# eddyxzc/lpopc

Measured on AMD Instinct MI355X. Metric: eval_g+eval_jac_g calls/sec, 4-phase 4096-LGR-pt problem, higher is better.
Workload: dtype f64

## Files before the change

lpopc_amd/csrc/rpm_ipm_device.hpp:

```cpp
#pragma once
#include <hip/hip_runtime.h>

#include "rpm_ipm.hpp"

namespace rpm {

constexpr int IPM_FMAX = 1024;
constexpr int IPM_TRACE = 8;
constexpr double IPM_INF = 1e19;
constexpr int IPM_LB_H = 6;
constexpr int IPM_LB_PART = 80 * 16;
constexpr int IPM_LB_SMALL = 8 + 2 * (2 * IPM_LB_H) * (2 * IPM_LB_H) + 2 * (2 * IPM_LB_H);

struct IpmOpts {
  double tol = 1e-8, mu_init = 0.1, kappa_eps = 10.0, kappa_mu = 0.2, theta_mu = 1.5, tau_min = 0.99;
  double bound_push = 1e-2, bound_frac = 1e-2, kappa_sigma = 1e10, s_max = 100.0;
  double ws_bound_push = 1e-3, ws_bound_frac = 1e-3, ws_slack_bound_push = 1e-3, ws_slack_bound_frac = 1e-3;
  double ws_mult_bound_push = 1e-3, ws_mult_init_max = 1e6;
  double gamma_theta = 1e-5, gamma_phi = 1e-8, eta_phi = 1e-8, delta = 1.0, s_theta = 1.1, s_phi = 2.3, gamma_alpha = 0.05;
  double delta_c = 1e-9, delta_w_first = 1e-4, delta_w_min = 1e-20, delta_w_max = 1e40, kw_inc_first = 100.0, kw_inc = 8.0,
         kw_dec = 1.0 / 3.0;
  int max_iter = 3000, max_ls = 40;
  double acceptable_tol = 1e-6;
  int acceptable_iter = 15;
// ... 35 lines not shown
struct IpmDev {
  int B, n, m, ns, nv, Nt, Nb, nb, b, CS, nnz_jac, nnz_h;
  long long sg, sv, kstride;
  const int *pos, *row_slack, *slack_row, *jac_dst, *hes_dst, *diag_dst, *slk_dst, *jt_ptr, *jt_ent, *jt_row;
  const int *hg_ptr, *hg_src, *hg_dst;
  int n_hg;
  const int *as_dst, *as_ki, *as_hg, *as_ptr;
  int as_nchunk;
  const int* long_cols;
  int n_long;
  const double *gl, *gu;
  double *v, *vl, *vu, *zL, *zU, *lam, *dv, *dlam, *dzL, *dzU, *glag, *c, *rhs, *K, *filt;
  double *xe, *xt, *grad, *g, *jac, *hess, *obj, *gt, *objt;
  double *vR, *dr2;
  double *vl0, *vu0;
  double *pp, *nn, *zp, *zn, *dpp, *dnn, *dzp, *dzn;
  double* rfilt;
  double* part;
  int* tick;
  double *dv2, *dlam2, *dzL2, *dzU2, *csoc, *ct;
  double* trace;
  int trace_cap;
  IpmInst* inst;
  int* cnt;
  IpmOpts o;
  const KktSub* subs;
  int n_sub, n_l1, n_l2;
  int* piv;
  const int *cg_ptr, *cg_src, *cg_dst;
  const int *rg_ptr, *rg_src, *rg_dst;
  const int *rs_dst, *rs_src;
  const int* gap_pos;
  int n_cg, n_rg, n_rs, n_gap;
  const int *cg2_ptr, *cg2_src, *cg2_dst, *rg2_ptr, *rg2_src, *rg2_dst, *rs2_dst, *rs2_src;
  int n_cg2, n_rg2, n_rs2;
  int n_cg_long, n_cg2_long;
  int max_sub_nt;
  int df_tiles;
  size_t l1_dense_lds;
  int last_dense_corner;
  size_t l2_dense_lds, last_dense_lds;
  int df_on;
  const int *df_ptr, *df_ki, *df_hg, *as_live;
  int as_nlive;
  const unsigned long long* df_map;
  int rhs_mult;
  int lb_on;
  double *lb_S, *lb_Y;
  double *lb_xprev;
  double *lb_gold;
  int scal_on;
  double *sc, *sf, *lam_h;
  const int* jac_row;
  int nnz_var;
  double *lb_small;
  double *lb_part;
  double *lb_Z;
};

constexpr int IPM_VEC_BLOCKS = 64;
constexpr int IPM_VEC_PART = 24;
constexpr int IPM_MT = 8;

void ipm_launch_set_state0(const IpmDev& D, int x_state0, int M, int nx, const double* d_state0, hipStream_t st);
void ipm_launch_init(const IpmDev& D, const double* d_x0, hipStream_t st, int warm = 0);
void ipm_launch_init_slack(const IpmDev& D, hipStream_t st, int warm = 0);
void ipm_launch_warm_duals(const IpmDev& D, const double* d_x0, const double* d_lambda, const double* d_zL, const double* d_zU, hipStream_t st);
void ipm_launch_bound_multipliers(const IpmDev& D, double* d_zL, double* d_zU, hipStream_t st);
void ipm_launch_pack_x(const IpmDev& D, hipStream_t st);
void ipm_launch_residual(const IpmDev& D, hipStream_t st);
void ipm_launch_assemble(const IpmDev& D, int nnz_max, hipStream_t st);
void ipm_launch_inertia(const IpmDev& D, hipStream_t st);
void ipm_launch_direction(const IpmDev& D, hipStream_t st);
void ipm_launch_trial(const IpmDev& D, hipStream_t st);
void ipm_launch_accept(const IpmDev& D, hipStream_t st);
void ipm_launch_update(const IpmDev& D, hipStream_t st);
void ipm_launch_soc_rhs(const IpmDev& D, hipStream_t st);
void ipm_launch_soc_direction(const IpmDev& D, hipStream_t st);
void ipm_launch_scaling_factors(const IpmDev& D, hipStream_t st);
void ipm_launch_scale(const IpmDev& D, double* g, double* jac, int jac0, int jac1, double* obj, double* grad, hipStream_t st);
void ipm_launch_scale_lambda(const IpmDev& D, hipStream_t st);
void ipm_launch_scale_hessian(const IpmDev& D, hipStream_t st);
void ipm_launch_unscale_lambda(const IpmDev& D, double* out, hipStream_t st);
void lb_launch_reset(const IpmDev& D, hipStream_t st);
void lb_launch_update(const IpmDev& D, hipStream_t st);
void lb_launch_columns_and_solve(const IpmDev& D, hipStream_t st);
// ... 15 lines not shown
```

lpopc_amd/csrc/rpm_ipm_solver.hip:

```cpp
#include <algorithm>
#include <cstdlib>
#include <cstring>
#include <memory>
#include <new>

#include "rpm_ipm_solver.hpp"

using namespace rpm;

namespace {
struct IpmAllocs {
  rpm_ipm* h;
  int rc = RPM_OK;
  template <class T>
  void room(T** dst, size_t count) { if (!rc) rc = ipm_alloc(h, dst, count); }
  template <class T>
  void table(const T** dst, const std::vector<T>& src) {
    T* p = nullptr;
    if (!rc) rc = ipm_alloc(h, &p, src.size(), src.data());
    *dst = p;
  }
};

bool env_is_zero(const char* name) {
// ... 45 lines not shown
  D.n_cg = int(p.cg_dst.size()); D.n_rg = int(p.rg_dst.size()); D.n_rs = int(p.rs_dst.size()); D.n_gap = int(p.gap_pos.size());
  a.table(&D.cg2_ptr, p.cg2_ptr); a.table(&D.cg2_src, p.cg2_src); a.table(&D.cg2_dst, p.cg2_dst);
  a.table(&D.rg2_ptr, p.rg2_ptr); a.table(&D.rg2_src, p.rg2_src); a.table(&D.rg2_dst, p.rg2_dst);
  a.table(&D.rs2_dst, p.rs2_dst); a.table(&D.rs2_src, p.rs2_src);
  D.n_cg2 = int(p.cg2_dst.size()); D.n_rg2 = int(p.rg2_dst.size()); D.n_rs2 = int(p.rs2_dst.size());
  D.n_cg_long = p.n_cg_long; D.n_cg2_long = p.n_cg2_long;
  return a.rc;
}

int alloc_state(rpm_ipm* h) {
  Engine& e = h->eng->e;
  const IpmPlan& p = h->plan;
  IpmDev& D = h->D;
  const size_t B = size_t(D.B), Bm = B * size_t(std::max(p.m, 1));
  IpmAllocs a{h};
  a.room(&D.v, B * p.nv); a.room(&D.vl, B * p.nv); a.room(&D.vu, B * p.nv);
  a.room(&D.zL, B * p.nv); a.room(&D.zU, B * p.nv); a.room(&D.lam, B * p.m);
  a.room(&D.dv, B * p.nv); a.room(&D.dlam, B * p.m); a.room(&D.dzL, B * p.nv);
  a.room(&D.dzU, B * p.nv); a.room(&D.glag, B * p.nv); a.room(&D.c, B * p.m);
  a.room(&D.rhs, B * size_t(p.Nt_alloc)); a.room(&D.K, B * size_t(p.storage())); a.room(&D.filt, B * 2 * IPM_FMAX);
  a.room(&D.xe, B * p.n); a.room(&D.xt, B * p.n); a.room(&D.grad, B * p.n);
  a.room(&D.g, B * size_t(D.sg)); a.room(&D.jac, B * size_t(D.sv)); a.room(&D.hess, B * size_t(e.nnz_h));
  a.room(&D.obj, B); a.room(&D.gt, B * size_t(D.sg)); a.room(&D.objt, B);
  a.room(&D.inst, B); a.room(&D.cnt, size_t(4));
  a.room(&D.vR, B * p.nv); a.room(&D.dr2, B * p.nv);
  a.room(&D.vl0, B * p.nv); a.room(&D.vu0, B * p.nv);
  if (h->lbfgs) {
    a.room(&D.lb_S, B * IPM_LB_H * p.n); a.room(&D.lb_Y, B * IPM_LB_H * p.n);
    a.room(&D.lb_xprev, B * p.n); a.room(&D.lb_gold, B * p.nv);
    a.room(&D.lb_small, B * IPM_LB_SMALL); a.room(&D.lb_part, B * IPM_LB_PART);
    a.room(&D.lb_Z, size_t(2 * IPM_LB_H) * B * size_t(p.Nt_alloc));
  }
  a.room(&D.sc, Bm); a.room(&D.sf, B); a.room(&D.lam_h, Bm);
  a.table(&D.jac_row, e.jac_i);
  D.nnz_var = e.nnz_nl + e.nnz_lin;
  a.room(&D.pp, Bm); a.room(&D.nn, Bm); a.room(&D.zp, Bm); a.room(&D.zn, Bm);
  a.room(&D.dpp, Bm); a.room(&D.dnn, Bm); a.room(&D.dzp, Bm); a.room(&D.dzn, Bm);
  a.room(&D.dlam2, Bm); a.room(&D.csoc, Bm); a.room(&D.ct, Bm);
  a.room(&D.dv2, B * p.nv); a.room(&D.dzL2, B * p.nv); a.room(&D.dzU2, B * p.nv);
  a.room(&D.rfilt, B * 2 * IPM_FMAX);
  a.room(&D.part, B * IPM_VEC_BLOCKS * IPM_VEC_PART); a.room(&D.tick, B);
  if (a.rc) return a.rc;
  if (hipMemsetAsync(D.tick, 0, B * sizeof(int), static_cast<hipStream_t>(dev_stream(e))) != hipSuccess) return device_failed(h, "hipMemset");
  if (hipHostMalloc(reinterpret_cast<void**>(&h->h_cnt), 4 * sizeof(int)) != hipSuccess) return device_failed(h, "hipHostMalloc");
  std::vector<double> l(B * p.nv, 0.0), u(B * p.nv, 0.0);
  for (size_t bi = 0; bi < B; ++bi)
    for (int i = 0; i < p.n; ++i) { l[bi * p.nv + i] = e.xl[i]; u[bi * p.nv + i] = e.xu[i]; }
  if (hipMemcpy(D.vl0, l.data(), l.size() * sizeof(double), hipMemcpyHostToDevice) != hipSuccess ||
      hipMemcpy(D.vu0, u.data(), u.size() * sizeof(double), hipMemcpyHostToDevice) != hipSuccess) return device_failed(h, "hipMemcpy");
  h->h_inst.resize(B);
  return RPM_OK;
}

int choose_kernels(rpm_ipm* h, const IpmSubList& s) {
  const IpmPlan& p = h->plan;
  IpmDev& D = h->D;
  const size_t B = size_t(D.B);
  D.last_dense_corner = 1;
  if (s.n_l1 > 0) {
    auto dense_lds_of = [&](int first, int count) -> size_t {
      int rows = 0;
      for (int i = first; i < first + count; ++i) rows = std::max(rows, s.subs[size_t(i)].g.block_rows());
      return count > 0 && rows <= kkt_factor_dense_max_block_rows() ? kkt_factor_dense_lds_bytes(rows) : 0;
    };
    h->l1_dense_lds = dense_lds_of(0, s.n_l1);
    h->l2_dense_lds = dense_lds_of(s.n_l1, s.n_l2);
    for (int i = s.n_l1; i < s.n_l1 + s.n_l2; ++i)
// ... 14 lines not shown
  if (p.max_rows > 4 * IPM_MT * 16) {
    h->err = "band + border of " + std::to_string(p.max_rows - IPM_W) + " rows exceeds the factorisation's 512 rows per block column";
    return RPM_E_UNSUPPORTED;
  }
  h->factor_lds = kkt_factor_lds_bytes(p);
  if (h->factor_lds > 150 * 1024) {
    h->err = "band of " + std::to_string(p.b) + " and border of " + std::to_string(p.nb) + " rows do not fit the factorisation's LDS";
    return RPM_E_UNSUPPORTED;
  }
  if (kkt_factor_prepare(h->factor_mt, h->factor_lds) != hipSuccess) return device_failed(h, "hipFuncSetAttribute");
  return RPM_OK;
}
}

extern "C" {

int rpm_ipm_create(rpm_engine* eng, rpm_ipm** out) {
  if (!eng || !out) return RPM_E_INVALID;
  *out = nullptr;
  Engine& e = eng->e;
  const bool lbfgs = e.hessian_mode != RPM_HESSIAN_EXACT;
  if (e.shard_world > 1) {
    e.err = "rpm_ipm_create: interval-sharded engines are not supported (shard instances across ranks instead)";
    return RPM_E_UNSUPPORTED;
  }
  if (!e.dev) {
    int rc = device_init(e, 0);
    if (rc) return rc;
  }
  int rc = lbfgs ? RPM_OK : ensure_hessian(e);
  if (rc) return rc;
  std::unique_ptr<rpm_ipm> h(new (std::nothrow) rpm_ipm);
  if (!h) return RPM_E_INVALID;
  h->eng = eng;
  h->lbfgs = lbfgs;
  e.ipm_attached += 1;
  h->attached = true;
  auto fail = [&e](int code, const std::string& why) { e.err = "rpm_ipm_create: " + why; return code; };

  std::string why;
  rc = build_ipm_plan(e, h->plan, &why, e.opt_ipm_nested != 0);
  if (e.opt_ipm_nested == -1 && (rc || h->plan.max_rows > 4 * IPM_MT * 16 || kkt_factor_lds_bytes(h->plan) > 150 * 1024))
    rc = build_ipm_plan(e, h->plan, &why, 0);
  if (rc) return fail(rc, why);
  const IpmPlan& p = h->plan;

// ... 411 lines not shown
```

lpopc_amd/csrc/rpm_ipm_solver.hpp:

```cpp
#pragma once
#include <algorithm>
#include <cstdio>
#include <string>
#include <vector>

#include "rpm_device_internal.hpp"
#include "rpm_ipm_device.hpp"

struct rpm_ipm {
  rpm_engine* eng = nullptr;
  rpm::IpmPlan plan;
  rpm::IpmDev D{};
  std::vector<void*> allocs;
  int* h_cnt = nullptr;
  size_t factor_lds = 0;
  size_t l1_dense_lds = 0;
  size_t l2_dense_lds = 0, last_dense_lds = 0;
  int factor_mt = rpm::IPM_MT;
  std::string err;
  std::vector<rpm::IpmInst> h_inst;
  int total_factorizations = 0, total_iterations = 0, total_trials = 0, total_soc = 0;
  hipEvent_t ev[4] = {nullptr, nullptr, nullptr, nullptr};
  double factor_ms = 0.0, solve_ms = 0.0;
  bool solve_pending = false;
// ... 46 lines not shown
  if (factor) kkt_launch_factor(h->D, h->factor_mt, h->factor_lds, st);
  if (solve) kkt_launch_solve(h->D, check_status, st, forward_done);
  return launch_check(h, "kkt kernels");
}

int ipm_check_start_args(rpm_ipm* h, const char* who, const char* need, bool warm, const void* x, const void* lambda, const void* z_L,
                         const void* z_U);
int ipm_start(rpm_ipm* h, bool warm, const double* d_x, const double* d_lambda, const double* d_zL, const double* d_zU, hipStream_t st);
int host_form(rpm_ipm* h, double** d_x, double** d_l, double** d_zL, double** d_zU);

inline int ipm_abi_status(int device_status) {
  return device_status == 1 ? 0 : (device_status == 6 ? 1 : device_status);
}

struct IpmLoop {
  rpm_ipm* h;
  Engine& e;
  IpmDev& D;
  hipStream_t st;
  bool scal;
  int eng_fail(int rc) const { h->err = e.err; return rc; }

  int fetch_counts() const {
    IPM_TRY(h, hipMemcpyAsync(h->h_cnt, D.cnt, 4 * sizeof(int), hipMemcpyDeviceToHost, st));
    IPM_TRY(h, hipStreamSynchronize(st));
    return RPM_OK;
  }
  int evaluate_and_residual() const {
    int rc;
    ipm_launch_pack_x(D, st);
    if ((rc = dev_eval_obj(e, D.xe, D.obj, D.grad, st))) return eng_fail(rc);
    if ((rc = dev_eval_cons(e, D.xe, D.g, D.jac, 3 | 4 | 16, st))) return eng_fail(rc);
    if (scal) ipm_launch_scale(D, D.g, D.jac, 0, D.nnz_var, D.obj, D.grad, st);
    IPM_TRY(h, hipMemsetAsync(D.cnt, 0, 4 * sizeof(int), st));
    ipm_launch_residual(D, st);
    if (h->lbfgs) lb_launch_update(D, st);
    return fetch_counts();
  }
  int exact_hessian() const {
    if (scal) ipm_launch_scale_lambda(D, st);
    if (int rc = dev_eval_h(e, D.xe, 1.0, scal ? D.lam_h : D.lam, D.hess, st)) return eng_fail(rc);
    if (scal) ipm_launch_scale_hessian(D, st);
    return RPM_OK;
  }
  int factor_with_inertia_correction() const {
    int rc;
    for (int tries = 0; tries < 80; ++tries) {
      IPM_TRY(h, hipMemsetAsync(D.cnt + 1, 0, sizeof(int), st));
      ipm_launch_assemble(D, std::max(e.nnz_jac, e.nnz_h), st);
      IPM_TRY(h, hipEventRecord(h->ev[0], st));
      if ((rc = factor_and_solve_launch(h, st, true, false, 1))) return rc;
      IPM_TRY(h, hipEventRecord(h->ev[1], st));
      ipm_launch_inertia(D, st);
      h->total_factorizations += 1;
      if ((rc = fetch_counts())) return rc;
      float ms = 0.f;
      if (hipEventElapsedTime(&ms, h->ev[0], h->ev[1]) == hipSuccess) h->factor_ms += ms;
      if (h->h_cnt[1] == 0) break;
    }
    return RPM_OK;
  }
  int substitute() const {
    IPM_TRY(h, hipEventRecord(h->ev[2], st));
    if (h->lbfgs && h->lb_iterations > 0) {
      lb_launch_columns_and_solve(D, st);
      lb_launch_small(D, st);
    }
    if (int rc = factor_and_solve_launch(h, st, false, true, 1, 1)) return rc;
    if (h->lbfgs) lb_launch_correct(D, 1, st);
    IPM_TRY(h, hipEventRecord(h->ev[3], st));
    h->solve_pending = true;
    return RPM_OK;
  }
  int direction() const {
    IPM_TRY(h, hipMemsetAsync(D.cnt + 2, 0, 2 * sizeof(int), st));
    ipm_launch_direction(D, st);
    h->h_cnt[3] = 0;
    return RPM_OK;
  }
  int line_search_round(double* soc_rhs_copy = nullptr) const {
    int rc;
    if (h->h_cnt[3] > 0) {
      ipm_launch_soc_rhs(D, st);
      if (soc_rhs_copy)
        IPM_TRY(h, hipMemcpyAsync(soc_rhs_copy, D.rhs, size_t(D.B) * size_t(h->plan.Nt_alloc) * sizeof(double), hipMemcpyDeviceToHost, st));
      if ((rc = factor_and_solve_launch(h, st, false, true, 2))) return rc;
      if (h->lbfgs) lb_launch_correct(D, 2, st);
      ipm_launch_soc_direction(D, st);
      h->total_soc += 1;
    }
    ipm_launch_trial(D, st);
    if ((rc = dev_eval_obj(e, D.xt, D.objt, nullptr, st))) return eng_fail(rc);
    if ((rc = dev_eval_cons(e, D.xt, D.gt, nullptr, 1 | 4, st))) return eng_fail(rc);
    if (scal) ipm_launch_scale(D, D.gt, nullptr, 0, 0, D.objt, nullptr, st);
    IPM_TRY(h, hipMemsetAsync(D.cnt + 2, 0, 2 * sizeof(int), st));
    ipm_launch_accept(D, st);
    h->total_trials += 1;
    if ((rc = fetch_counts())) return rc;
    if (h->solve_pending) {
      float ms = 0.f;
      if (hipEventElapsedTime(&ms, h->ev[2], h->ev[3]) == hipSuccess) h->solve_ms += ms;
      h->solve_pending = false;
    }
    return RPM_OK;
  }
  bool line_search_over() const { return h->h_cnt[2] == 0 && h->h_cnt[3] == 0; }
  int line_search() const {
    int rc;
    if ((rc = direction())) return rc;
    for (int ls = 0; ls <= D.o.max_ls + D.o.max_soc + 2; ++ls) {
      if ((rc = line_search_round())) return rc;
      if (line_search_over()) break;
    }
    return RPM_OK;
  }
  int update() const {
    ipm_launch_update(D, st);
    if (h->lbfgs) {
// ... 39 lines not shown
```

lpopc_amd/csrc/rpm_ipm_step_kernels.hip:

```cpp
#include <algorithm>
#include <cmath>
#include <cstring>
#include <new>

#include "rpm_device_internal.hpp"
#include "rpm_ipm_device.hpp"

namespace rpm {

__device__ inline double block_red(double v, int kind, double* sh) {
  for (int o = 32; o; o >>= 1) {
    const double w = __shfl_down(v, o);
    v = kind == 0 ? v + w : (kind == 1 ? fmax(v, w) : fmin(v, w));
  }
  __syncthreads();
  if ((threadIdx.x & 63) == 0) sh[threadIdx.x >> 6] = v;
  __syncthreads();
  double r = sh[0];
  for (int i = 1; i < int(blockDim.x >> 6); ++i) r = kind == 0 ? r + sh[i] : (kind == 1 ? fmax(r, sh[i]) : fmin(r, sh[i]));
  return r;
}
__device__ inline bool has_lo(double l, double u) { return l > -IPM_INF && l != u; }
__device__ inline bool has_up(double l, double u) { return u < IPM_INF && l != u; }

// ... 214 lines not shown
  if (S.status != 0) return;
  const double *lam = D.lam + size_t(bi) * D.m, *jac = D.jac + size_t(bi) * D.sv;
  const bool resto = S.mode == 2;
  if (int(blockIdx.x) >= n_thread_blocks) {
    const int i = D.long_cols[blockIdx.x - n_thread_blocks];
    double acc = 0.0;
    for (int q = D.jt_ptr[i] + threadIdx.x; q < D.jt_ptr[i + 1]; q += blockDim.x) acc += jac[D.jt_ent[q]] * lam[D.jt_row[q]];
    acc = block_red(acc, 0, sh);
    if (threadIdx.x == 0) D.glag[size_t(bi) * D.nv + i] = (resto ? 0.0 : D.grad[size_t(bi) * D.n + i]) + acc;
    return;
  }
  const int i = blockIdx.x * blockDim.x + threadIdx.x;
  if (i >= D.nv) return;
  double acc;
  if (i < D.n) {
    if (D.jt_ptr[i + 1] - D.jt_ptr[i] > IPM_LONG_COLUMN) return;
    acc = resto ? 0.0 : D.grad[size_t(bi) * D.n + i];
    for (int q = D.jt_ptr[i]; q < D.jt_ptr[i + 1]; ++q) acc += jac[D.jt_ent[q]] * lam[D.jt_row[q]];
  } else {
    acc = -lam[D.slack_row[i - D.n]];
  }
  D.glag[size_t(bi) * D.nv + i] = acc;
}
__global__ __launch_bounds__(1024) void ipm_residual_kernel(IpmDev D) {
  __shared__ double sh[16];
  __shared__ int verdict;
  const int bi = blockIdx.y, t = threadIdx.x, i0 = blockIdx.x * blockDim.x + threadIdx.x, stride = gridDim.x * blockDim.x;
  IpmInst& S = D.inst[bi];
  if (S.status != 0) return;
  const int mode_in = S.mode;
  if (mode_in == 3) {
    if (t == 0 && blockIdx.x == 0) { S.refactor = 1; S.delta_w = 0.0; atomicAdd(&D.cnt[0], 1); }
    return;
  }
  const double *v = D.v + size_t(bi) * D.nv, *vl = D.vl + size_t(bi) * D.nv, *vu = D.vu + size_t(bi) * D.nv;
  const double *zL = D.zL + size_t(bi) * D.nv, *zU = D.zU + size_t(bi) * D.nv, *lam = D.lam + size_t(bi) * D.m;
  const double *g = D.g + size_t(bi) * D.sg, *glag = D.glag + size_t(bi) * D.nv;
  double dinf = 0, cinf = 0, th1 = 0, cmax = 0, cmin = 1e300, sl = 0, sz = 0, ln = 0, bad = 0, nzb = 0;
  double csq = 0, dsq = 0, psum = 0, psq = 0, nfree = 0;
  double cinf_u = 0;
  #pragma unroll 4
  for (int r = i0; r < D.m; r += stride) {
    const int s = D.row_slack[r];
    const double glr = D.scal_on ? D.sc[size_t(bi) * D.m + r] * D.gl[r] : D.gl[r];
    const double cr = s < 0 ? g[r] - glr : g[r] - v[D.n + s];
    D.c[size_t(bi) * D.m + r] = cr;
    if (!(fabs(cr) < 1e300)) bad = 1;
    cinf = fmax(cinf, fabs(cr));
    cinf_u = fmax(cinf_u, D.scal_on ? fabs(cr / D.sc[size_t(bi) * D.m + r]) : fabs(cr));
    th1 += fabs(cr);
    csq += cr * cr;
  }
  if (mode_in == 2) {
    const IpmOpts& o = D.o;
    const double rho = o.resto_rho, zeta = S.zeta;
// ... 29 lines not shown
      verdict = 0;
      if (bad != 0 || !(fabs(f) < 1e300) || !(fabs(ln) < 1e300) || !(fabs(lnpn) < 1e300)) { S.status = 5; verdict = 2; }
      else {
        const double phi_o = f - S.mu * ln;
        bool back = S.resto_it > 0 && th1 <= o.kappa_resto * S.th0 && th1 <= S.theta_max;
        const double* F = D.filt + size_t(bi) * 2 * IPM_FMAX;
        for (int k = 0; back && k < S.nfilt; ++k)
          if (th1 >= F[2 * k] && phi_o >= F[2 * k + 1]) back = false;
        if (back) verdict = 1;
        else if (S.resto_it >= o.resto_max) { S.status = 3; verdict = 2; }
        else if (S.iter >= o.max_iter) { S.status = 2; verdict = 2; }
        else {
          if (S.resto_it == 0) { S.thr_max = 1e4 * fmax(1.0, thr); S.thr_min = 1e-4 * fmax(1.0, thr); }
          double mu_r = S.mu_r;
          bool stuck;
          if (monotone_mu(o, dinf, rinf, cmax, cmin, true, 1.0, o.tol / 10.0, &mu_r, &stuck)) S.nrfilt = 0;
          if (stuck) { S.status = 3; verdict = 2; }
          else {
            S.mu_r = mu_r; S.zeta = sqrt(mu_r); S.tau = fmax(o.tau_min, 1.0 - mu_r);
            S.f = f; S.theta = th1; S.lnsum = ln; S.cinf = cinf; S.th_r = thr;
            S.phi_r = rho * spn + 0.5 * S.zeta * qd - mu_r * (ln + lnpn);
            S.refactor = 1;
            S.delta_w = 0.0;
            atomicAdd(&D.cnt[0], 1);
          }
        }
      }
    }
    __syncthreads();
    if (verdict != 1) return;
    #pragma unroll 4
    for (int i = t; i < D.nv; i += blockDim.x) {
      const double l = vl[i], u = vu[i];
      if (l == u) continue;
      const size_t o2 = size_t(bi) * D.nv + i;
      if (l > -IPM_INF) D.zL[o2] = reset16(fmin(D.zL[o2], 1e3), v[i] - l, S.mu, D.o.kappa_sigma);
      if (u < IPM_INF) D.zU[o2] = reset16(fmin(D.zU[o2], 1e3), u - v[i], S.mu, D.o.kappa_sigma);
    }
    if (t == 0) { S.mode = 3; S.refactor = 1; S.delta_w = 0.0; atomicAdd(&D.cnt[0], 1); }
    return;
  }
  #pragma unroll 4
  for (int i = i0; i < D.nv; i += stride) {
    const double acc = glag[i];
    const double l = vl[i], u = vu[i], vi = v[i], zli = zL[i], zui = zU[i];
    if (l != u) {
      const double dres = acc - zli + zui;
      dinf = fmax(dinf, fabs(dres));
      dsq += dres * dres; nfree += 1;
      if (!(fabs(acc) < 1e300)) bad = 1;
      if (l > -IPM_INF) {
        const double d = vi - l, pr = zli * d;
        cmax = fmax(cmax, pr); cmin = fmin(cmin, pr); sz += zli; ln += log(d); nzb += 1; psum += pr; psq += pr * pr;
      }
      if (u < IPM_INF) {
        const double d = u - vi, pr = zui * d;
        cmax = fmax(cmax, pr); cmin = fmin(cmin, pr); sz += zui; ln += log(d); nzb += 1; psum += pr; psq += pr * pr;
      }
    }
  }
  #pragma unroll 4
  for (int r = i0; r < D.m; r += stride) sl += fabs(lam[r]);
// ... 32 lines not shown
      S.fixed_mode = 0;
      if (S.nrefs < 4) S.refs[S.nrefs++] = kkt_err;
      else { S.refs[0] = S.refs[1]; S.refs[1] = S.refs[2]; S.refs[2] = S.refs[3]; S.refs[3] = kkt_err; }
      const double xi = cmin / avg, fac = fmin(0.05 * (1.0 - xi) / xi, 2.0);
      mu_new = fmax(mu_min, fmin(0.1 * fac * fac * fac * avg, S.mu_max));
    } else if (!S.fixed_mode) {
      S.fixed_mode = 1;
      mu_new = fmax(mu_min, fmin(o.mu_init_factor * avg, S.mu_max));
    }
    if (mu_new >= 0.0) {
      if (mu_new != mu) S.nfilt = 0;
      mu = mu_new;
      from_oracle = true;
    }
  }
  bool at_floor;
  if (!from_oracle && monotone_mu(o, dinf / sd, cinf, cmax, cmin, nzb > 0, sc, mu_min, &mu, &at_floor)) S.nfilt = 0;
  S.mu = mu;
  S.tau = fmax(o.tau_min, 1.0 - mu);
  S.phi = S.f - mu * ln;
  S.refactor = 1;
  S.delta_w = 0.0;
  if (o.ic_hot && S.ic_hot && o.kw_dec * S.delta_w_last >= o.ic_hot_min) S.delta_w = o.kw_dec * S.delta_w_last;
  atomicAdd(&D.cnt[0], 1);
}

__device__ inline double ftb(double w, double dw, double tau, double a) { return dw < 0 ? fmin(a, -tau * w / dw) : a; }

__device__ inline double bound_step(double s, double z, double d, bool upper, double mu, double tau, double* amax, double* az, double* gphi) {
  const double dz = mu / s - z - z / s * d;
  *amax = ftb(s, d, tau, *amax);
  *az = ftb(z, dz, tau, *az);
  *gphi = upper ? *gphi + mu / s : *gphi - mu / s;
  return dz;
}
__device__ inline void newton_step_unknowns(const IpmDev& D, int bi, const double* sol, double* dv, double* dzL, double* dzU, double mu, double tau,
                                            bool resto, double zeta, double* amax_io, double* az_io, double* dphi_io, double* bad_io) {
  const size_t o = size_t(bi) * D.nv;
  const int i0 = blockIdx.x * blockDim.x + threadIdx.x, stride = gridDim.x * blockDim.x;
  double amax = *amax_io, az = *az_io, dphi = *dphi_io, bad = *bad_io;
  #pragma unroll 4
  for (int i = i0; i < D.nv; i += stride) {
    const double l = D.vl[o + i], u = D.vu[o + i], vi = D.v[o + i], dsol = sol[D.pos[i]], zl = D.zL[o + i], zu = D.zU[o + i];
    const double gri = resto ? zeta * D.dr2[o + i] * (vi - D.vR[o + i]) : (i < D.n ? D.grad[size_t(bi) * D.n + i] : 0.0);
    double d = 0.0, dl = 0.0, du = 0.0;
    if (l != u) {
      d = dsol;
// ... 50 lines not shown
  }
  if (mode == 2) {
    const double rho = D.o.resto_rho, zeta = S.zeta;
    double amax = 1.0, az = 1.0, dphi = 0.0, bad = 0.0;
    newton_step_unknowns(D, bi, sol, D.dv, D.dzL, D.dzU, mu, tau, true, zeta, &amax, &az, &dphi, &bad);
    #pragma unroll 4
    for (int r = i0; r < D.m; r += stride) {
      const double pp = D.pp[om + r], nn = D.nn[om + r], zp = D.zp[om + r], zn = D.zn[om + r], lam = D.lam[om + r];
      const double sp = zp / pp, sn = zn / nn, dlam = sol[D.pos[D.nv + r]];
      if (!(fabs(dlam) < 1e300)) bad = 1;
      const double rp = rho - lam - mu / pp, rn = rho + lam - mu / nn;
      const double dp = (dlam - rp) / sp, dn = (-dlam - rn) / sn;
      double gp = rho, gn = rho;
      const double dzp = bound_step(pp, zp, dp, false, mu, tau, &amax, &az, &gp), dzn = bound_step(nn, zn, dn, false, mu, tau, &amax, &az, &gn);
      dphi += gp * dp + gn * dn;
      D.dlam[om + r] = dlam; D.dpp[om + r] = dp; D.dnn[om + r] = dn; D.dzp[om + r] = dzp; D.dzn[om + r] = dzn;
    }
    if (!reduce_and_combine(D, bi, sh, red_min(amax), red_min(az), red_sum(dphi), red_max(bad))) return;
    if (t != 0) return;
    if (bad != 0) { S.status = 5; return; }
    S.alpha_max = amax; S.alpha_z = az; S.alpha = amax; S.dphi = dphi;
    S.alpha_min = alpha_min23(D.o, S.th_r, S.thr_min, dphi);
    S.ls = 0; S.accepted = 0; S.armijo = 0; S.soc_on = 0; S.soc_req = 0; S.use_soc = 0;
    atomicAdd(&D.cnt[2], 1);
    return;
  }
  double amax, az, dphi, bad;
  if (!newton_step(D, bi, sol, D.dv, D.dlam, D.dzL, D.dzU, mu, tau, sh, &amax, &az, &dphi, &bad)) return;
  if (t != 0) return;
  if (bad != 0) { S.status = 5; return; }
  S.alpha_max = amax; S.alpha_z = az; S.alpha = amax; S.dphi = dphi;
  S.alpha_min = alpha_min23(D.o, S.theta, S.theta_min, dphi);
  S.ls = 0; S.accepted = 0; S.armijo = 0; S.soc_on = 0; S.soc_req = 0; S.use_soc = 0; S.soc_p = 0;
  atomicAdd(&D.cnt[2], 1);
}

__global__ void ipm_soc_rhs_kernel(IpmDev D) {
  const int bi = blockIdx.y;
  const IpmInst& S = D.inst[bi];
  if (S.status != 0 || !S.soc_req) return;
  const size_t o = size_t(bi) * D.nv, om = size_t(bi) * D.m;
  const int stride = gridDim.x * blockDim.x, t0 = blockIdx.x * blockDim.x + threadIdx.x;
  double* rhs = D.rhs + size_t(bi) * D.Nt;
  const bool first = S.soc_p == 0;
  const double mix = first ? S.alpha : S.alpha_soc, mu = S.mu;
  for (int r = t0; r < D.m; r += stride) {
    const double cs = mix * (first ? D.c[om + r] : D.csoc[om + r]) + D.ct[om + r];
    D.csoc[om + r] = cs;
    rhs[D.pos[D.nv + r]] = -cs;
  }
  for (int i = t0; i < D.nv; i += stride) {
    const double l = D.vl[o + i], u = D.vu[o + i];
    double r = 0.0;
    if (l != u) {
      r = D.glag[o + i];
      if (l > -IPM_INF) r -= mu / (D.v[o + i] - l);
      if (u < IPM_INF) r += mu / (u - D.v[o + i]);
// ... 15 lines not shown
  S.soc_req = 0;
  if (bad != 0) { S.soc_on = 0; S.alpha = 0.5 * S.alpha; S.ls += 1; return; }
  S.alpha_soc = amax; S.az_soc = az;
}

__device__ inline bool filter_accepts(const IpmOpts& op, double theta, double theta_min, double theta_max, double phi, double dphi, double th,
                                      double phit, double a_test, bool dominated, double bad, bool* armijo) {
  const double slack = 10.0 * 2.220446049250313e-16 * fabs(phi);
  *armijo = false;
  if (bad != 0 || !(th <= theta_max) || dominated) return false;
  const bool sw = dphi < 0 && a_test * pow(-dphi, op.s_phi) > op.delta * pow(theta, op.s_theta);
  if (theta <= theta_min && sw) return *armijo = phit - phi - op.eta_phi * a_test * dphi <= slack;
  return th <= (1.0 - op.gamma_theta) * theta || phit - (phi - op.gamma_phi * theta) <= slack;
}
__global__ void ipm_trial_kernel(IpmDev D) {
  const int bi = blockIdx.y;
  const IpmInst& S = D.inst[bi];
  if (S.status != 0 || S.accepted || S.enter_resto) return;
  const int i = blockIdx.x * blockDim.x + threadIdx.x;
  if (i >= D.n) return;
  const size_t o = size_t(bi) * D.nv + i;
  D.xt[size_t(bi) * D.n + i] = S.soc_on ? D.v[o] + S.alpha_soc * D.dv2[o] : D.v[o] + S.alpha * D.dv[o];
}
__global__ __launch_bounds__(1024) void ipm_accept_kernel(IpmDev D) {
  __shared__ double sh[16];
  const int bi = blockIdx.y, t = threadIdx.x, i0 = blockIdx.x * blockDim.x + threadIdx.x, stride = gridDim.x * blockDim.x;
  IpmInst& S = D.inst[bi];
  const int go = S.status == 0 && !S.accepted && !S.enter_resto, mode = S.mode, soc = S.soc_on;
  const double a = soc ? S.alpha_soc : S.alpha;
  __syncthreads();
  if (!go) return;
  const size_t o = size_t(bi) * D.nv, om = size_t(bi) * D.m;
  const double* dvp = soc ? D.dv2 : D.dv;
  double th = 0.0, ln = 0.0, bad = 0.0, qd = 0.0, spn = 0.0, lnpn = 0.0;
  const bool resto = mode == 2;
  #pragma unroll 4
  for (int i = i0; i < D.nv; i += stride) {
    const double l = D.vl[o + i], u = D.vu[o + i], vi = D.v[o + i], di = dvp[o + i];
    if (l == u) continue;
    const double vt = vi + a * di;
    if (l > -IPM_INF) ln += log(vt - l);
    if (u < IPM_INF) ln += log(u - vt);
    if (resto) { const double dd = vt - D.vR[o + i]; qd += D.dr2[o + i] * dd * dd; }
  }
  #pragma unroll 4
  for (int r = i0; r < D.m; r += stride) {
    const int s = D.row_slack[r];
// ... 13 lines not shown
  if (!reduce_and_combine(D, bi, sh, red_sum(th), red_sum(ln), red_max(bad), red_sum(qd, resto), red_sum(spn, resto),
                          red_sum(lnpn, resto))) return;
  const IpmOpts& op = D.o;
  const double phit_all = resto ? op.resto_rho * spn + 0.5 * S.zeta * qd - S.mu_r * (ln + lnpn) : D.objt[bi] - S.mu * ln;
  double dom = 0.0;
  {
    const double* F = (resto ? D.rfilt : D.filt) + size_t(bi) * 2 * IPM_FMAX;
    const int nf = resto ? S.nrfilt : S.nfilt;
    for (int k = t; k < nf; k += blockDim.x)
      if (th >= F[2 * k] && phit_all >= F[2 * k + 1]) dom = 1.0;
  }
  const bool dominated = block_red(dom, 1, sh) != 0.0;
  if (t != 0) return;
  S.th_trial = th; S.phi_trial = phit_all;
  if (resto) {
    if (!(fabs(phit_all) < 1e300)) bad = 1;
    bool armijo;
    const bool ok = filter_accepts(op, S.th_r, S.thr_min, S.thr_max, S.phi_r, S.dphi, th, phit_all, a, dominated, bad, &armijo);
    if (armijo) S.armijo = 1;
    if (ok) { S.accepted = 1; return; }
    S.alpha = 0.5 * a;
    S.ls += 1;
    if (S.alpha < S.alpha_min || S.ls > op.max_ls) { S.status = 3; return; }
    atomicAdd(&D.cnt[2], 1);
    return;
  }
  const double ft = D.objt[bi];
  if (!(fabs(ft) < 1e300) || !(fabs(ln) < 1e300)) bad = 1;
  bool armijo;
  const bool ok = filter_accepts(op, S.theta, S.theta_min, S.theta_max, S.phi, S.dphi, th, phit_all, S.alpha, dominated, bad, &armijo);
  if (armijo) S.armijo = 1;
  if (ok) {
    S.accepted = 1;
    if (soc) { S.use_soc = 1; S.n_soc += 1; }
    return;
  }
  const bool th_ok = fabs(th) < 1e300 && bad == 0;
  if (soc) {
    if (th_ok && S.soc_p + 1 < op.max_soc && th <= op.kappa_soc * S.th_old_soc) {
      S.soc_p += 1; S.th_old_soc = th; S.soc_req = 1;
      atomicAdd(&D.cnt[3], 1);
      return;
    }
    S.soc_on = 0;
  } else if (S.ls == 0 && op.max_soc > 0 && th_ok && th >= S.theta) {
    S.soc_on = 1; S.soc_p = 0; S.th_old_soc = S.theta; S.soc_req = 1;
    atomicAdd(&D.cnt[3], 1);
    return;
  }
  S.alpha = 0.5 * S.alpha;
  S.ls += 1;
  if (S.alpha < S.alpha_min || S.ls > op.max_ls) {
    if (S.err0 <= op.acceptable_tol) S.status = 6;
    else if (op.resto && S.theta > op.tol) S.enter_resto = 1;
    else if (op.resto && S.n_recalc < 3) S.enter_resto = 2;
    else S.status = 3;
    return;
  }
  atomicAdd(&D.cnt[2], 1);
}

__device__ inline void filter_append(double* F, int* n, double theta, double phi, const IpmOpts& o) {
  if (*n >= IPM_FMAX) return;
  F[2 * *n] = (1.0 - o.gamma_theta) * theta;
  F[2 * *n + 1] = phi - o.gamma_phi * theta;
  *n += 1;
}
__device__ inline void trace_record(const IpmDev& D, int bi, const IpmInst& S, double mu, double a, double az, double delta_w, double ls) {
  if (!D.trace || S.iter >= D.trace_cap) return;
  double* R = D.trace + (size_t(bi) * D.trace_cap + S.iter) * IPM_TRACE;
  R[0] = S.f; R[1] = S.theta; R[2] = mu; R[3] = a; R[4] = az; R[5] = delta_w; R[6] = S.err0; R[7] = ls;
}
__device__ inline void apply_step(const IpmDev& D, int bi, const double* dv, const double* dlam, const double* dzL, const double* dzU, double a,
                                  double az, double mu) {
  const int i0 = blockIdx.x * blockDim.x + threadIdx.x, stride = gridDim.x * blockDim.x;
  const size_t o = size_t(bi) * D.nv, om = size_t(bi) * D.m;
  const double ks = D.o.kappa_sigma;
  #pragma unroll 4
  for (int i = i0; i < D.nv; i += stride) {
    const double l = D.vl[o + i], u = D.vu[o + i], v0 = D.v[o + i], di = dv[o + i];
    const double zl = D.zL[o + i], zu = D.zU[o + i], dl = dzL[o + i], du = dzU[o + i];
    if (l == u) continue;
// ... 206 lines not shown
```

lpopc_amd/csrc/rpm_kkt_solve.hip:

```cpp
#include <algorithm>
#include <cmath>
#include <cstring>
#include <new>

#include "rpm_device_internal.hpp"
#include "rpm_ipm_device.hpp"

namespace rpm {

__device__ inline void block_range(const KktGeom& G, int J0, int* J1, int* nrb, int* nr) {
  if (J0 < G.Nb) {
    *J1 = min(J0 + IPM_W, G.Nb);
    const int last = min(*J1 - 1 + G.b, G.Nb - 1);
    *nrb = max(last - *J1 + 1, 0);
    *nr = *nrb + G.nb;
  } else {
    *J1 = min(J0 + IPM_W, G.Nt);
    *nrb = 0;
    *nr = G.Nt - *J1;
  }
}
__device__ inline int panel_row(const KktGeom& G, int J0, int J1, int nrb, int q) {
  return J0 >= G.Nb ? J1 + q : (q < nrb ? J1 + q : G.Nb + (q - nrb));
}
// ... 106 lines not shown
    }
    SOLVE_BARRIER();
    if (t < W) zs[t] = t < B.w ? r[B.J0 + t] / Dg[t * (W + 1) + t] - (red[0][t] + red[1][t] + red[2][t] + red[3][t]) : 0.0;
    SOLVE_BARRIER();
    if (t < B.w) {
      double x = zs[t];
#pragma unroll
      for (int k = 0; k < W; ++k)
        if (k > t && k < B.w) x = __builtin_fma(Dg[k * (W + 1) + t], zs[k], x);
      r[B.J0 + t] = x;
    }
    SOLVE_BARRIER();
  };
  if (bwd_begin > 0) { fetch(bwd_begin - 1, dg0, l0); if (PF == 2) fetch(bwd_begin - 2, dg1, l1); }
  for (int blk = bwd_begin - 1; blk >= 0; blk -= PF) {
    backward_step(blk, dg0, l0);
    if (PF == 2 && blk - 1 >= 0) backward_step(blk - 1, dg1, l1);
  }
  if (RL)
    for (int i = t; i < G.Nt; i += nt) rg[i] = rsh[i];
#undef SOLVE_BARRIER
}

__global__ __launch_bounds__(256) void ipm_inertia_kernel(IpmDev D) {
  const int bi = (blockIdx.x * blockDim.x + threadIdx.x) >> 6, lane = threadIdx.x & 63;
  if (bi >= D.B) return;
  IpmInst& S = D.inst[bi];
  if (S.status != 0 || !S.refactor) return;
  const IpmOpts& o = D.o;
  int np = 0, nn = 0, nz = 0;
  for (int s2 = lane; s2 < D.n_sub; s2 += 64) {
    const int* q = D.piv + (size_t(bi) * D.n_sub + s2) * 3;
    np += q[0]; nn += q[1]; nz += q[2];
  }
  for (int w = 32; w; w >>= 1) { np += __shfl_xor(np, w); nn += __shfl_xor(nn, w); nz += __shfl_xor(nz, w); }
  if (lane != 0) return;
  S.npos = np; S.nneg = nn; S.nbad = nz;
  if (S.npos == D.nv && S.nbad == 0) {
    S.refactor = 0;
    if (S.delta_w > 0) S.delta_w_last = S.delta_w;
    if (S.mode == 0) S.ic_hot = S.delta_w > 0;
    return;
  }
  if (S.delta_w == 0.0) S.delta_w = S.delta_w_last == 0.0 ? o.delta_w_first : fmax(o.delta_w_min, o.kw_dec * S.delta_w_last);
  else S.delta_w *= S.delta_w_last == 0.0 ? o.kw_inc_first : o.kw_inc;
  if (S.delta_w > o.delta_w_max) { S.status = 4; return; }
  atomicAdd(&D.cnt[1], 1);
}

__global__ __launch_bounds__(256) void kkt_gather_seq_kernel(double* vall, long long vstride, const int* __restrict__ ptr, const int* __restrict__ src,
                                                             const int* __restrict__ dst, int n, const IpmInst* inst, int check_status, int kmod) {
  const int bi = blockIdx.y, bk = bi % kmod;
  if (check_status && (inst[bk].status != 0 || (check_status == 2 && !inst[bk].soc_req))) return;
  double* v = vall + size_t(bi) * vstride;
  const int lane = threadIdx.x & 63, wave = (blockIdx.x * blockDim.x + threadIdx.x) >> 6, n_waves = (gridDim.x * blockDim.x) >> 6;
  for (int i = wave; i < n; i += n_waves) {
    const int j0 = ptr[i], j1 = ptr[i + 1];
    double acc = v[dst[i]];
    for (int j = j0; j < j1; j += 64) {
      const double mine = j + lane < j1 ? v[src[j + lane]] : 0.0;
      const int m = min(64, j1 - j);
      for (int k = 0; k < m; ++k) acc += __shfl(mine, k, 64);
    }
    if (lane == 0) v[dst[i]] = acc;
  }
}
__global__ void kkt_vec_kernel(double* vall, long long vstride, const int* __restrict__ dst, const int* __restrict__ src, int n, int mode,
                               const IpmInst* inst, int check_status, int kmod) {
  const int bi = blockIdx.y, bk = bi % kmod;
  if (check_status && (inst[bk].status != 0 || (check_status == 2 && !inst[bk].soc_req) || (check_status == 3 && !inst[bk].refactor))) return;
// ... 57 lines not shown
```

Before: 743,200.

## Publish per-step counters to mapped host memory from the last workgroup

Control counters now accumulate in per-workgroup shared memory and are merged through one packed 64-bit atomic ticket. The last workgroup to finish writes the totals straight into mapped pinned host memory with system-scope stores. This removes the per-step hipMemsetAsync calls and the device-to-host memcpy before each stream sync. The cost is a ticket atomic per workgroup and a new cap on instance count set by the field width. The benchmarked eval_g/eval_jac_g path is probably not touched by these kernels.

```diff
diff --git a/lpopc_amd/csrc/rpm_ipm_device.hpp b/lpopc_amd/csrc/rpm_ipm_device.hpp
--- a/lpopc_amd/csrc/rpm_ipm_device.hpp
+++ b/lpopc_amd/csrc/rpm_ipm_device.hpp
@@ -81,7 +81,8 @@
   double* trace;
   int trace_cap;
   IpmInst* inst;
-  int* cnt;
+  int* cnt_host;
+  unsigned long long* cnt_tick;
   IpmOpts o;
   const KktSub* subs;
   int n_sub, n_l1, n_l2;
@@ -121,6 +122,31 @@
 constexpr int IPM_VEC_PART = 24;
 constexpr int IPM_MT = 8;
 
+constexpr int IPM_CNT_BITS = 21;
+constexpr int IPM_CNT_MAX = 1 << IPM_CNT_BITS;
+#ifdef __HIPCC__
+__device__ inline void ipm_counts_begin(unsigned* wg) {
+  if (threadIdx.x < 2) wg[threadIdx.x] = 0;
+  __syncthreads();
+}
+__device__ inline void ipm_count(unsigned* wg, int slot) { atomicAdd(&wg[slot], 1u); }
+__device__ inline void ipm_host_word(const IpmDev& D, int k, int value) {
+  __hip_atomic_store(&D.cnt_host[k], value, __ATOMIC_RELAXED, __HIP_MEMORY_SCOPE_SYSTEM);
+}
+__device__ inline bool ipm_counts_to_host(const IpmDev& D, const unsigned* wg, int first, int n_slots) {
+  __syncthreads();
+  if (threadIdx.x != 0) return false;
+  constexpr unsigned long long field = (1ull << IPM_CNT_BITS) - 1;
+  const unsigned long long mine = (1ull << (2 * IPM_CNT_BITS)) | ((unsigned long long)wg[1] << IPM_CNT_BITS) | wg[0];
+  const unsigned long long all = atomicAdd(D.cnt_tick, mine) + mine;
+  if ((all >> (2 * IPM_CNT_BITS)) != (unsigned long long)gridDim.x * gridDim.y) return false;
+  *D.cnt_tick = 0;
+  ipm_host_word(D, first, int(all & field));
+  if (n_slots > 1) ipm_host_word(D, first + 1, int((all >> IPM_CNT_BITS) & field));
+  return true;
+}
+#endif
+
 void ipm_launch_set_state0(const IpmDev& D, int x_state0, int M, int nx, const double* d_state0, hipStream_t st);
 void ipm_launch_init(const IpmDev& D, const double* d_x0, hipStream_t st, int warm = 0);
 void ipm_launch_init_slack(const IpmDev& D, hipStream_t st, int warm = 0);
diff --git a/lpopc_amd/csrc/rpm_ipm_solver.hip b/lpopc_amd/csrc/rpm_ipm_solver.hip
--- a/lpopc_amd/csrc/rpm_ipm_solver.hip
+++ b/lpopc_amd/csrc/rpm_ipm_solver.hip
@@ -91,7 +91,7 @@
   a.room(&D.xe, B * p.n); a.room(&D.xt, B * p.n); a.room(&D.grad, B * p.n);
   a.room(&D.g, B * size_t(D.sg)); a.room(&D.jac, B * size_t(D.sv)); a.room(&D.hess, B * size_t(e.nnz_h));
   a.room(&D.obj, B); a.room(&D.gt, B * size_t(D.sg)); a.room(&D.objt, B);
-  a.room(&D.inst, B); a.room(&D.cnt, size_t(4));
+  a.room(&D.inst, B); a.room(&D.cnt_tick, size_t(1));
   a.room(&D.vR, B * p.nv); a.room(&D.dr2, B * p.nv);
   a.room(&D.vl0, B * p.nv); a.room(&D.vu0, B * p.nv);
   if (h->lbfgs) {
@@ -111,7 +111,10 @@
   a.room(&D.part, B * IPM_VEC_BLOCKS * IPM_VEC_PART); a.room(&D.tick, B);
   if (a.rc) return a.rc;
   if (hipMemsetAsync(D.tick, 0, B * sizeof(int), static_cast<hipStream_t>(dev_stream(e))) != hipSuccess) return device_failed(h, "hipMemset");
-  if (hipHostMalloc(reinterpret_cast<void**>(&h->h_cnt), 4 * sizeof(int)) != hipSuccess) return device_failed(h, "hipHostMalloc");
+  if (hipMemsetAsync(D.cnt_tick, 0, sizeof(unsigned long long), static_cast<hipStream_t>(dev_stream(e))) != hipSuccess) return device_failed(h, "hipMemset");
+  if (hipHostMalloc(reinterpret_cast<void**>(&h->h_cnt), 4 * sizeof(int), hipHostMallocMapped) != hipSuccess) return device_failed(h, "hipHostMalloc");
+  if (hipHostGetDevicePointer(reinterpret_cast<void**>(&D.cnt_host), h->h_cnt, 0) != hipSuccess) return device_failed(h, "hipHostGetDevicePointer");
+  h->h_cnt[0] = h->h_cnt[1] = h->h_cnt[2] = h->h_cnt[3] = 0;
   std::vector<double> l(B * p.nv, 0.0), u(B * p.nv, 0.0);
   for (size_t bi = 0; bi < B; ++bi)
     for (int i = 0; i < p.n; ++i) { l[bi * p.nv + i] = e.xl[i]; u[bi * p.nv + i] = e.xu[i]; }
@@ -172,6 +175,10 @@
   const bool lbfgs = e.hessian_mode != RPM_HESSIAN_EXACT;
   if (e.shard_world > 1) {
     e.err = "rpm_ipm_create: interval-sharded engines are not supported (shard instances across ranks instead)";
+    return RPM_E_UNSUPPORTED;
+  }
+  if (e.n_instances >= IPM_CNT_MAX) {
+    e.err = "rpm_ipm_create: at most " + std::to_string(IPM_CNT_MAX - 1) + " instances (the counts' fields, rpm_ipm_device.hpp)";
     return RPM_E_UNSUPPORTED;
   }
   if (!e.dev) {
diff --git a/lpopc_amd/csrc/rpm_ipm_solver.hpp b/lpopc_amd/csrc/rpm_ipm_solver.hpp
--- a/lpopc_amd/csrc/rpm_ipm_solver.hpp
+++ b/lpopc_amd/csrc/rpm_ipm_solver.hpp
@@ -92,7 +92,6 @@
   int eng_fail(int rc) const { h->err = e.err; return rc; }
 
   int fetch_counts() const {
-    IPM_TRY(h, hipMemcpyAsync(h->h_cnt, D.cnt, 4 * sizeof(int), hipMemcpyDeviceToHost, st));
     IPM_TRY(h, hipStreamSynchronize(st));
     return RPM_OK;
   }
@@ -102,7 +101,6 @@
     if ((rc = dev_eval_obj(e, D.xe, D.obj, D.grad, st))) return eng_fail(rc);
     if ((rc = dev_eval_cons(e, D.xe, D.g, D.jac, 3 | 4 | 16, st))) return eng_fail(rc);
     if (scal) ipm_launch_scale(D, D.g, D.jac, 0, D.nnz_var, D.obj, D.grad, st);
-    IPM_TRY(h, hipMemsetAsync(D.cnt, 0, 4 * sizeof(int), st));
     ipm_launch_residual(D, st);
     if (h->lbfgs) lb_launch_update(D, st);
     return fetch_counts();
@@ -116,7 +114,6 @@
   int factor_with_inertia_correction() const {
     int rc;
     for (int tries = 0; tries < 80; ++tries) {
-      IPM_TRY(h, hipMemsetAsync(D.cnt + 1, 0, sizeof(int), st));
       ipm_launch_assemble(D, std::max(e.nnz_jac, e.nnz_h), st);
       IPM_TRY(h, hipEventRecord(h->ev[0], st));
       if ((rc = factor_and_solve_launch(h, st, true, false, 1))) return rc;
@@ -143,7 +140,6 @@
     return RPM_OK;
   }
   int direction() const {
-    IPM_TRY(h, hipMemsetAsync(D.cnt + 2, 0, 2 * sizeof(int), st));
     ipm_launch_direction(D, st);
     h->h_cnt[3] = 0;
     return RPM_OK;
@@ -163,7 +159,6 @@
     if ((rc = dev_eval_obj(e, D.xt, D.objt, nullptr, st))) return eng_fail(rc);
     if ((rc = dev_eval_cons(e, D.xt, D.gt, nullptr, 1 | 4, st))) return eng_fail(rc);
     if (scal) ipm_launch_scale(D, D.gt, nullptr, 0, 0, D.objt, nullptr, st);
-    IPM_TRY(h, hipMemsetAsync(D.cnt + 2, 0, 2 * sizeof(int), st));
     ipm_launch_accept(D, st);
     h->total_trials += 1;
     if ((rc = fetch_counts())) return rc;
diff --git a/lpopc_amd/csrc/rpm_ipm_step_kernels.hip b/lpopc_amd/csrc/rpm_ipm_step_kernels.hip
--- a/lpopc_amd/csrc/rpm_ipm_step_kernels.hip
+++ b/lpopc_amd/csrc/rpm_ipm_step_kernels.hip
@@ -260,7 +260,7 @@
   }
   D.glag[size_t(bi) * D.nv + i] = acc;
 }
-__global__ __launch_bounds__(1024) void ipm_residual_kernel(IpmDev D) {
+__device__ __forceinline__ void residual_body(const IpmDev& D, unsigned* wg) {
   __shared__ double sh[16];
   __shared__ int verdict;
   const int bi = blockIdx.y, t = threadIdx.x, i0 = blockIdx.x * blockDim.x + threadIdx.x, stride = gridDim.x * blockDim.x;
@@ -268,7 +268,7 @@
   if (S.status != 0) return;
   const int mode_in = S.mode;
   if (mode_in == 3) {
-    if (t == 0 && blockIdx.x == 0) { S.refactor = 1; S.delta_w = 0.0; atomicAdd(&D.cnt[0], 1); }
+    if (t == 0 && blockIdx.x == 0) { S.refactor = 1; S.delta_w = 0.0; ipm_count(wg, 0); }
     return;
   }
   const double *v = D.v + size_t(bi) * D.nv, *vl = D.vl + size_t(bi) * D.nv, *vu = D.vu + size_t(bi) * D.nv;
@@ -344,7 +344,7 @@
             S.phi_r = rho * spn + 0.5 * S.zeta * qd - mu_r * (ln + lnpn);
             S.refactor = 1;
             S.delta_w = 0.0;
-            atomicAdd(&D.cnt[0], 1);
+            ipm_count(wg, 0);
           }
         }
       }
@@ -359,7 +359,7 @@
       if (l > -IPM_INF) D.zL[o2] = reset16(fmin(D.zL[o2], 1e3), v[i] - l, S.mu, D.o.kappa_sigma);
       if (u < IPM_INF) D.zU[o2] = reset16(fmin(D.zU[o2], 1e3), u - v[i], S.mu, D.o.kappa_sigma);
     }
-    if (t == 0) { S.mode = 3; S.refactor = 1; S.delta_w = 0.0; atomicAdd(&D.cnt[0], 1); }
+    if (t == 0) { S.mode = 3; S.refactor = 1; S.delta_w = 0.0; ipm_count(wg, 0); }
     return;
   }
   #pragma unroll 4
@@ -438,7 +438,13 @@
   S.refactor = 1;
   S.delta_w = 0.0;
   if (o.ic_hot && S.ic_hot && o.kw_dec * S.delta_w_last >= o.ic_hot_min) S.delta_w = o.kw_dec * S.delta_w_last;
-  atomicAdd(&D.cnt[0], 1);
+  ipm_count(wg, 0);
+}
+__global__ __launch_bounds__(1024) void ipm_residual_kernel(IpmDev D) {
+  __shared__ unsigned wg[2];
+  ipm_counts_begin(wg);
+  residual_body(D, wg);
+  if (ipm_counts_to_host(D, wg, 0, 1)) ipm_host_word(D, 1, 0), ipm_host_word(D, 2, 0), ipm_host_word(D, 3, 0);
 }
 
 __device__ inline double ftb(double w, double dw, double tau, double a) { return dw < 0 ? fmin(a, -tau * w / dw) : a; }
@@ -535,7 +541,6 @@
     S.alpha_max = amax; S.alpha_z = az; S.alpha = amax; S.dphi = dphi;
     S.alpha_min = alpha_min23(D.o, S.th_r, S.thr_min, dphi);
     S.ls = 0; S.accepted = 0; S.armijo = 0; S.soc_on = 0; S.soc_req = 0; S.use_soc = 0;
-    atomicAdd(&D.cnt[2], 1);
     return;
   }
   double amax, az, dphi, bad;
@@ -545,7 +550,6 @@
   S.alpha_max = amax; S.alpha_z = az; S.alpha = amax; S.dphi = dphi;
   S.alpha_min = alpha_min23(D.o, S.theta, S.theta_min, dphi);
   S.ls = 0; S.accepted = 0; S.armijo = 0; S.soc_on = 0; S.soc_req = 0; S.use_soc = 0; S.soc_p = 0;
-  atomicAdd(&D.cnt[2], 1);
 }
 
 __global__ void ipm_soc_rhs_kernel(IpmDev D) {
@@ -607,7 +611,7 @@
   const size_t o = size_t(bi) * D.nv + i;
   D.xt[size_t(bi) * D.n + i] = S.soc_on ? D.v[o] + S.alpha_soc * D.dv2[o] : D.v[o] + S.alpha * D.dv[o];
 }
-__global__ __launch_bounds__(1024) void ipm_accept_kernel(IpmDev D) {
+__device__ __forceinline__ void accept_body(const IpmDev& D, unsigned* wg) {
   __shared__ double sh[16];
   const int bi = blockIdx.y, t = threadIdx.x, i0 = blockIdx.x * blockDim.x + threadIdx.x, stride = gridDim.x * blockDim.x;
   IpmInst& S = D.inst[bi];
@@ -667,7 +671,7 @@
     S.alpha = 0.5 * a;
     S.ls += 1;
     if (S.alpha < S.alpha_min || S.ls > op.max_ls) { S.status = 3; return; }
-    atomicAdd(&D.cnt[2], 1);
+    ipm_count(wg, 0);
     return;
   }
   const double ft = D.objt[bi];
@@ -684,13 +688,13 @@
   if (soc) {
     if (th_ok && S.soc_p + 1 < op.max_soc && th <= op.kappa_soc * S.th_old_soc) {
       S.soc_p += 1; S.th_old_soc = th; S.soc_req = 1;
-      atomicAdd(&D.cnt[3], 1);
+      ipm_count(wg, 1);
       return;
     }
     S.soc_on = 0;
   } else if (S.ls == 0 && op.max_soc > 0 && th_ok && th >= S.theta) {
     S.soc_on = 1; S.soc_p = 0; S.th_old_soc = S.theta; S.soc_req = 1;
-    atomicAdd(&D.cnt[3], 1);
+    ipm_count(wg, 1);
     return;
   }
   S.alpha = 0.5 * S.alpha;
@@ -702,7 +706,13 @@
     else S.status = 3;
     return;
   }
-  atomicAdd(&D.cnt[2], 1);
+  ipm_count(wg, 0);
+}
+__global__ __launch_bounds__(1024) void ipm_accept_kernel(IpmDev D) {
+  __shared__ unsigned wg[2];
+  ipm_counts_begin(wg);
+  accept_body(D, wg);
+  ipm_counts_to_host(D, wg, 2, 2);
 }
 
 __device__ inline void filter_append(double* F, int* n, double theta, double phi, const IpmOpts& o) {
diff --git a/lpopc_amd/csrc/rpm_kkt_solve.hip b/lpopc_amd/csrc/rpm_kkt_solve.hip
--- a/lpopc_amd/csrc/rpm_kkt_solve.hip
+++ b/lpopc_amd/csrc/rpm_kkt_solve.hip
@@ -152,7 +152,7 @@
 #undef SOLVE_BARRIER
 }
 
-__global__ __launch_bounds__(256) void ipm_inertia_kernel(IpmDev D) {
+__device__ __forceinline__ void inertia_body(const IpmDev& D, unsigned* wg) {
   const int bi = (blockIdx.x * blockDim.x + threadIdx.x) >> 6, lane = threadIdx.x & 63;
   if (bi >= D.B) return;
   IpmInst& S = D.inst[bi];
@@ -175,7 +175,13 @@
   if (S.delta_w == 0.0) S.delta_w = S.delta_w_last == 0.0 ? o.delta_w_first : fmax(o.delta_w_min, o.kw_dec * S.delta_w_last);
   else S.delta_w *= S.delta_w_last == 0.0 ? o.kw_inc_first : o.kw_inc;
   if (S.delta_w > o.delta_w_max) { S.status = 4; return; }
-  atomicAdd(&D.cnt[1], 1);
+  ipm_count(wg, 0);
+}
+__global__ __launch_bounds__(256) void ipm_inertia_kernel(IpmDev D) {
+  __shared__ unsigned wg[2];
+  ipm_counts_begin(wg);
+  inertia_body(D, wg);
+  ipm_counts_to_host(D, wg, 1, 1);
 }
 
 __global__ __launch_bounds__(256) void kkt_gather_seq_kernel(double* vall, long long vstride, const int* __restrict__ ptr, const int* __restrict__ src,
```

New measurement: 739,500. About the same (-0.5%).
